# DiltheyLab/HLA-LA

Measured on AMD Instinct MI355X. Metric: paired reads/sec aligned to PRG graph, higher is better.
Workload: dtype int32

## Files before the change

hla-la_amd/__init__.py:

```python
from __future__ import annotations

import ctypes as C
import os

import numpy as np

_HERE = os.path.dirname(os.path.abspath(__file__))
LIB_PATH = os.environ.get("HLALA_LIB_PATH") or os.path.join(_HERE, "libhlala_gpu.so")

c_i32p = C.POINTER(C.c_int32)
c_i64p = C.POINTER(C.c_int64)
c_u8p = C.POINTER(C.c_uint8)
c_u32p = C.POINTER(C.c_uint32)
c_f64p = C.POINTER(C.c_double)

CHAIN_OK, CHAIN_SKIP_STRAND, CHAIN_SKIP_DUP = 0, 1, 2
CHAIN_ERR_COLUMNS, CHAIN_ERR_FRONTIER, CHAIN_ERR_INPUT = -1, -2, -3


class GraphDesc(C.Structure):
    _fields_ = [("n_levels", C.c_int32), ("n_nodes", C.c_int32), ("n_edges", C.c_int32),
                ("node_level", c_i32p), ("edge_from", c_i32p), ("edge_to", c_i32p), ("edge_label", c_u8p)]


# ... 163 lines not shown
    return _filter_call(lambda *a: fn(ctx.h, *a), "hlala_filter_positions_gpu", ctx.last_error, e, params, raw)


def filter_gpu_times(ctx, enable=True):
    ms = (C.c_double * 6)()
    ctx.lib.hlala_filter_gpu_times.argtypes = [C.c_void_p, C.c_int, C.POINTER(C.c_double)]
    if ctx.lib.hlala_filter_gpu_times(ctx.h, int(bool(enable)), ms) != 0:
        raise HlalaError("hlala_filter_gpu_times failed")
    return dict(zip(("mapq_keys", "sort_scan", "first20", "reads", "coverage", "use"), (float(x) for x in ms)))


def host_filter_model(e, params=None, tie_rule=0, raw=False):
    h = _host_lib()
    fn = h.hlala_host_filter_model
    fn.argtypes = [C.POINTER(ExonPositionsOut), C.POINTER(FilterParams), c_u8p, c_u8p, C.POINTER(FilterStats), C.POINTER(C.c_int64), C.c_int32]; fn.restype = C.c_int
    h.hlala_host_last_error.restype = C.c_char_p
    return _filter_call(lambda *a: fn(*a, int(tie_rule)), "hlala_host_filter_model", lambda: h.hlala_host_last_error().decode(errors="replace"), e, params, raw)


CALL_ORDER_MAX_HEAP = 4096
CALL_ORDER_TILE = 1024
CALL_ORDER_COUNTS = ("path", "levels", "tile_ranges", "largest_tile", "heap_sorts", "largest_heap", "bytes_up", "bytes_down")
CALL_ORDER_HOST, CALL_ORDER_DEVICE, CALL_ORDER_REFUSED_NAN, CALL_ORDER_REFUSED_HEAP, CALL_ORDER_REFUSED_ALLOC = range(5)


def call_order_params():
    v = [C.c_int32() for _ in range(4)]
    h = _host_lib(); h.hlala_host_pair_order_params.restype = None
    h.hlala_host_pair_order_params(*[C.byref(x) for x in v])
    return dict(zip(("tile", "max_heap", "block", "chunk"), (x.value for x in v)))


def _pair_order_call(call, what, last_error, ll, ma, raw):
    a = [np.ascontiguousarray(x, np.float64) for x in (ll, ma)]
    n = len(a[0]); assert len(a[1]) == n
    order = np.full(max(1, n), -7, np.int32); cn = (C.c_int64 * 8)()
    rc = call(n, a[0].ctypes.data_as(c_f64p), a[1].ctypes.data_as(c_f64p), order.ctypes.data_as(c_i32p), cn)
    out = (order[:n], dict(zip(CALL_ORDER_COUNTS, (int(x) for x in cn))))
    if raw:
        return (int(rc), last_error() if rc != 0 else "") + out
    if rc != 0:
        err = HlalaError(f"{what} failed ({rc}): {last_error()}"); err.code = int(rc)
        raise err
    return out


# ... 1362 lines not shown
```

hla-la_amd/csrc/batch.h:

```cpp
#pragma once
#include "device_common.h"

namespace hlala {

template <template <class> class Ptr> struct DevBatchT {
    int n_pairs, n_reads, n_chains, stride;
    int from_seeds;
    int unpaired;
    Ptr<const int> read_off;
    Ptr<const uint8_t> read_bases;
    Ptr<const uint8_t> read_quals;
    Ptr<const int> chain_off;
    Ptr<const int> read_primary;
    Ptr<const int> chain_read;
    Ptr<const int> chain_contig;
    Ptr<const int> chain_pos;
    Ptr<const int> chain_offset;
    Ptr<const int> chain_as;
    Ptr<const uint8_t> chain_reverse;
    Ptr<const int> cigar_off;
    Ptr<const u32> cigar;
    Ptr<int> seed_status;
    Ptr<int> seed_ncols;
    Ptr<int> seed_begin;
// ... 31 lines not shown
    Ptr<uint8_t> strands_valid;
    Ptr<uint8_t> sel_mapq;
    Ptr<u64> counters;
    Ptr<int> work_counter;
    Ptr<int> retry_list;
    Ptr<int> pair_multi;
    Ptr<uint8_t> pair_deferred;
    Ptr<int> chain_order;
    Ptr<int> chain_bucket;
    Ptr<int> order_hist;
    int order_shift, order_nb;
    int long_chunk_nodes, long_max_segs;
    int order_cost;
    Ptr<int> chain_row;
    int n_rows;
    Ptr<int> dp_blk;
    Ptr<int> dp_list;
    int dp_nblk;
    int dp_band;
    int dp_band_risky;
    int dp_band_nodes;
    int dp_jf;
    int dp_long;
    Ptr<void> dp_items;
    Ptr<int> dbg;
};
typedef DevBatchT<HostP> DevBatch;
typedef DevBatchT<GlobP> DevBatchG;
static_assert(sizeof(DevBatch) == sizeof(DevBatchG), "one layout");
__device__ __forceinline__ const DevBatchG& dev_view(const DevBatch* p) { return *(const DevBatchG*)p; }
enum { DESC_VALUE = 0, DESC_VIEW = 1, DESC_GENERIC = 2 };
template <int FORM, class D> __device__ __forceinline__ decltype(auto) desc_of(const D& byValue, const D* inMemory)
{
    if constexpr (FORM == DESC_VIEW) return dev_view(inMemory);
    else if constexpr (FORM == DESC_GENERIC) return (*inMemory);
    else return (byValue);
}

template <class BT> __device__ __forceinline__ int ordered_chains(const BT& B) { return B.chain_order ? __builtin_amdgcn_readfirstlane(B.order_hist[B.order_nb - 1]) : B.n_chains; }

template <class BT> __device__ __forceinline__ size_t row_base(const BT& B, int c) { return (size_t)(B.chain_row ? B.chain_row[c] : c) * (size_t)B.stride; }

enum { DPL_BAND16 = 0, DPL_BAND32 = 2, DPL_BAND64 = 4, DPL_JF = 6, DPL_GEN = 10, DPL_N = 14 };
__host__ __device__ inline int dpl_list(int cls, int dir, bool isLong)
{
    if(cls >= 2) return (cls == 2 ? DPL_BAND16 : (cls == 3 ? DPL_BAND32 : DPL_BAND64)) + dir;
// ... 18 lines not shown
```

hla-la_amd/csrc/hlala_api.hip:

```cpp
#include <cmath>
#include <cstdio>
#include <cstring>
#include <cstdlib>
#include <algorithm>
#include <atomic>
#include <map>
#include <mutex>
#include <chrono>
#include <thread>
#include <set>
#include <string>
#include <unordered_map>
#include <vector>

#include "../../include/hlala_gpu.h"
#include "batch.h"
#include "flat_graph.hpp"
#include "host_internal.h"

#include "kernel_dp.hip"
#include "kernel_project.hip"
#include "kernel_order.hip"
#include "kernel_pair.hip"
#include "kernel_pair_overflow.hip"
// ... 42 lines not shown
    hlala_params params{};
    FlatGraph F;
    DevGraph G{};
    DevGraph* dG = nullptr;
    DevTables* dT = nullptr;
    double* d_islog = nullptr;
    long long* d_contig_off = nullptr; uint8_t* d_contig_seq = nullptr; int* d_contig_level = nullptr;
    int n_contigs = 0; std::vector<long long> contig_off;
    std::vector<void*> allocs;
    std::unordered_map<void*, size_t> block_bytes;
    std::multimap<size_t, void*> pool;
    size_t pool_bytes = 0;
    size_t pool_cap = (size_t)176 << 30;
    std::mutex pool_mu;
    std::set<struct hlala_batch*> batches;
    int dp_long_bases = 48;
    int jf_margin = 16;
    int stitch_by_row = 1;
    int stitch_draw = 12;
    bool side_after_pair = false;
    bool rows_all = false;
    bool band_risky = false;
    bool band_nodes = true;
    int band_grid = 0, band_margin = 8;
    DpClass dp[DP_LAST_TIER + 1]; DpClass dp_jf;
    int stitch_grid = 0;
    char* proj_slabs = nullptr; size_t proj_slab_bytes = 0; int proj_grid = 0, pair_grid = 0, pair_lean_grid = 0;
    char* rethread_slabs = nullptr; size_t rethread_slab_bytes = 0; int rethread_grid = 0;
    double* pair_scratch = nullptr;
    char* pair_over_slabs = nullptr; long long pair_over_scratch = 0, pair_over_slab_bytes = 0;
    char* proj_long_slabs = nullptr; size_t proj_long_slab_bytes = 0;
    void* create_scratch = nullptr; size_t create_scratch_bytes = 0; bool create_scratch_pinned = false;
    int long_chunk_nodes = 1 << 20, long_max_segs = 1 << 20;
    int order_cost = 0;
    int order_shift = 8, order_nb = 0;
    int* dbg_host = nullptr;
    int* d_cov = nullptr; int n_cov = 0; int* d_gene_first = nullptr; int* d_gene_last = nullptr; int n_genes = 0;
    struct KeptReads { uint8_t* store = nullptr; long long* start = nullptr; int* length = nullptr; int n = 0; };
    std::vector<KeptReads> kept;
    bool flt_timed = false; double flt_ms[6] = {0, 0, 0, 0, 0, 0};
    bool ord_gpu = false, ord_timed = false; int64_t ord_counts[HLALA_CALL_ORDER_COUNTS] = {0, 0, 0, 0, 0, 0, 0, 0}; double ord_ms[4] = {0, 0, 0, 0};
    std::string err;
};

enum BatchEvent {
    EV_PROJECT_BEGIN, EV_PROJECT_END, EV_EXTEND_BEGIN, EV_EXTEND_END, EV_PAIR_BEGIN, EV_PAIR_END,
// ... 24 lines not shown
    uint32_t first_chain = 0;
    float ms[3] = {0, 0, 0};
};

struct DevGuard {
    int prev = -1, want = -1;
    explicit DevGuard(int device) : want(device) { if(device >= 0 && hipGetDevice(&prev) == hipSuccess && prev != device) (void)hipSetDevice(device); else prev = -1; }
    ~DevGuard() { if(prev >= 0 && prev != want) (void)hipSetDevice(prev); }
    DevGuard(const DevGuard&) = delete; DevGuard& operator=(const DevGuard&) = delete;
};
#define DEV_GUARD(c) DevGuard dev_guard_((c) ? (c)->device : -1)

#define HIP_TRY(ctx, call) do { hipError_t e_ = (call); if(e_ != hipSuccess) { (ctx)->err = std::string(#call) + ": " + hipGetErrorString(e_); return HLALA_E_DEVICE; } } while(0)
#define HIP_TRY_F(ctx, call, cleanup) do { hipError_t e_ = (call); if(e_ != hipSuccess) { (ctx)->err = std::string(#call) + ": " + hipGetErrorString(e_); return cleanup(HLALA_E_DEVICE); } } while(0)

template<class C, int TIER> static void launch_dp(hlala_ctx* c, const DpClass& k, hipStream_t ws, hlala_batch* b, const DpPoolArgs& pool)
{
    hipLaunchKernelGGL((k_dp<C, TIER>), dim3(k.grid), dim3(k.block), 0, ws, c->dG, b->dB, (DpItem*)b->B.dp_items, k.slabs, k.slab_bytes, c->params.rng_seed + 2u * b->first_chain,
                       c->G.nrec_out, c->G.nrec_in, b->B.read_bases, pool);
}
template<class C, int TIER> static DpClass dp_class(int grid, size_t slab_bytes, const char* name) { return DpClass{grid, C::THREADS, nullptr, slab_bytes, name, launch_dp<C, TIER>}; }

static int flush_tail(hlala_ctx* c);
static int join_side(hlala_ctx* c, hlala_batch* b)
{
    if(b->tail_pooled) { int rf = flush_tail(c); if(rf) return rf; }
    if(b->side_inflight) {
        HIP_TRY(c, hipStreamWaitEvent(c->stream, b->ev[EV_DONE], 0));
        if(b->ev[EV_MAIN]) { HIP_TRY(c, hipEventRecord(b->ev[EV_MAIN], c->stream)); b->mainValid = true; b->side_inflight = false; }
    }
    return HLALA_OK;
}
static int batch_events(hlala_ctx* c, hlala_batch* b)
{
    if(b->eventsMade) return HLALA_OK;
    for(int i = 0; i < EV_N; i++) HIP_TRY(c, hipEventCreateWithFlags(&b->ev[i], i < EV_TIMED_N ? hipEventDefault : hipEventDisableTiming));
    b->eventsMade = true;
    return HLALA_OK;
}
static int mark_main(hlala_ctx* c, hlala_batch* b) { HIP_TRY(c, hipEventRecord(b->ev[EV_MAIN], c->stream)); b->mainValid = true; return HLALA_OK; }
struct ReaderScope {
    hlala_ctx* c; int rc = HLALA_OK;
    ReaderScope(hlala_ctx* c_, hlala_batch* b) : c(c_)
    {
        if(!c) return;
        if(b && b->tail_pooled) { rc = flush_tail(c); if(rc) return; }
// ... 258 lines not shown
        rc = dev_upload(c, c->allocs, contigs->contig_seq, total, &c->d_contig_seq); if(rc) return fail(rc);
        rc = dev_upload(c, c->allocs, contigs->contig_level, total, &c->d_contig_level); if(rc) return fail(rc);
    }
    rc = build_tables(c); if(rc) return fail(rc);
    rc = dev_upload(c, c->allocs, &c->G, 1, &c->dG); if(rc) return fail(rc);
    hipDeviceProp_t prop;
    if(hipGetDeviceProperties(&prop, device) != hipSuccess) { c->err = "hipGetDeviceProperties failed"; return fail(HLALA_E_DEVICE); }
    int cus = prop.multiProcessorCount > 0 ? prop.multiProcessorCount : 256;
    auto slab_pool = [&](char** out, size_t bytes, const char* what) -> int {
        if(device_malloc_retry(c->device, nullptr, (void**)out, bytes) != hipSuccess) { c->err = std::string("hipMalloc(") + what + ") failed"; return HLALA_E_DEVICE; }
        c->allocs.push_back(*out);
        if(hipMemsetAsync(*out, 0, bytes, c->active) != hipSuccess) { c->err = std::string("hipMemset(") + what + ") failed"; return HLALA_E_DEVICE; }
        return 0;
    };
    c->band_grid = cus * 20;
    if(const char* e = getenv("HLALA_DP_BAND")) { if(atoi(e) == 0) c->band_grid = 0; }
    if(const char* e = getenv("HLALA_DP_BAND_RISKY")) c->band_risky = atoi(e) != 0;
    if(const char* e = getenv("HLALA_DP_BAND_NODES")) c->band_nodes = atoi(e) != 0;
    if(const char* e = getenv("HLALA_ROWS_ALL")) c->rows_all = atoi(e) != 0;
    if(const char* e = getenv("HLALA_SIDE_AFTER_PAIR")) c->side_after_pair = atoi(e) != 0;
    if(const char* e = getenv("HLALA_POOL_CAP_GB")) { const long g = atol(e); if(g >= 0 && g <= 1024) c->pool_cap = (size_t)g << 30; }
    if(const char* e = getenv("HLALA_DP_BAND_MARGIN")) { const int m = atoi(e); if(m >= 0 && m <= 24) c->band_margin = m; }
    if(const char* e = getenv("HLALA_DP_JF_MARGIN")) { const int m = atoi(e); if(m >= 0 && m <= 200) c->jf_margin = m; }
    if(const char* e = getenv("HLALA_DP_LONG_BASES")) { const int m = atoi(e); if(m >= 0 && m <= 4096) c->dp_long_bases = m; }
    c->stitch_grid = cus * 20;
    if(const char* e = getenv("HLALA_STITCH_BY_ROW")) c->stitch_by_row = atoi(e) != 0;
    const size_t extBytes = std::max(dp_slab_bytes<DpSmall>(), dp_slab_bytes<DpWide>()), largeBytes = std::max(dp_slab_bytes<DpLarge>(), dp_slab_bytes<DpBroad>());
    DpClass* const dp = c->dp;
    c->dp_jf = dp_class<DpTinyJF, 0>(cus * 4 * DpTinyJF::WAVES, dp_slab_bytes<DpTiny>(), "k_dp<DpTinyJF>");
    dp[0] = dp_class<DpTiny, 0>(cus * 4 * DpTiny::WAVES, dp_slab_bytes<DpTiny>(), "k_dp<DpTiny>");
    dp[1] = dp_class<DpMid, 1>(cus * 16, dp_slab_bytes<DpMid>(), "k_dp<DpMid>");
    dp[2] = dp_class<DpSmall, 2>(cus * 20, extBytes, "k_dp<DpSmall>");
    dp[3] = dp_class<DpWide, 3>(cus * 7, extBytes, "k_dp<DpWide>");
    dp[4] = dp_class<DpBroad, 4>(cus * 3, largeBytes, "k_dp<DpBroad>");
    dp[5] = dp_class<DpLarge, 5>(cus, largeBytes, "k_dp<DpLarge>");
    dp[6] = dp_class<DpHuge, 6>(cus / 4 > 0 ? cus / 4 : 1, dp_inmemory_bytes<DpHuge>(), "k_dp<DpHuge>");
    if((rc = slab_pool(&dp[0].slabs, dp[0].slab_bytes * (size_t)(64 / DpTiny::GW) * (size_t)std::max(dp[0].grid, c->dp_jf.grid), "16-lane DP slabs"))) return fail(rc);
    c->dp_jf.slabs = dp[0].slabs;
    if((rc = slab_pool(&dp[1].slabs, dp[1].slab_bytes * (size_t)(64 / DpMid::GW) * (size_t)dp[1].grid, "32-lane DP slabs"))) return fail(rc);
    if((rc = slab_pool(&dp[2].slabs, extBytes * (size_t)dp[2].grid, "64-lane DP slabs"))) return fail(rc);
    if((rc = slab_pool(&dp[3].slabs, extBytes * (size_t)dp[3].grid, "wide-class DP slabs"))) return fail(rc);
    if((rc = slab_pool(&dp[4].slabs, largeBytes * (size_t)(dp[4].grid + dp[5].grid), "large-class DP slabs"))) return fail(rc);
    dp[5].slabs = dp[4].slabs + largeBytes * (size_t)dp[4].grid;
    if((rc = slab_pool(&dp[6].slabs, dp[6].slab_bytes * (size_t)dp[6].grid, "in-memory DP class"))) return fail(rc);
    c->proj_grid = cus * (c->params.max_columns <= PROJ_CAP_SHORT ? 12 : 8); c->pair_grid = cus * 16; c->pair_lean_grid = cus * 24;
    { int rcp = dev_alloc(c, c->allocs, (size_t)2 * c->pair_grid * PAIR_COMB, &c->pair_scratch, false); if(rcp) return fail(rcp); }
// ... 94 lines not shown
static int batch_alloc_outputs(hlala_ctx* c, hlala_batch* b)
{
    DevBatch& B = b->B;
    size_t nc = (size_t)B.n_chains, nr = (size_t)B.n_reads, np = (size_t)B.n_pairs;
    if(!b->prepared) { B.n_rows = B.n_chains; B.chain_row = nullptr; }
    size_t rowsAlloc = (size_t)(B.n_rows > 0 ? B.n_rows : 1);
    if(b->prepared && nc >= 4096) { const size_t gran = nc / 64; rowsAlloc = (rowsAlloc + gran - 1) / gran * gran; if(rowsAlloc > nc) rowsAlloc = nc; }
    const size_t cs = rowsAlloc * (size_t)B.stride;
    int rc = 0;
#define AL(field, n, zero) do { rc = dev_alloc(c, b->allocs, (n), &B.field, zero); if(rc) return rc; } while(0)
    if(!b->prepared) { AL(seed_status, nc, true); AL(seed_ncols, nc, true); }
    AL(seed_begin, nc, true); AL(seed_end, nc, true); AL(seed_removed, nc, true);
    AL(seed_level, cs, false); AL(seed_edge, cs, false); AL(seed_g, cs, false); AL(seed_s, cs, false);
    AL(ext_status, nc, true); AL(ext_ncols, nc, true); AL(ext_begin, nc, true); AL(ext_end, nc, true); AL(ext_ll, nc, true);
    AL(dp_iters, 2 * nc, true); AL(dp_score, 2 * nc, true); AL(dp_ncols, 2 * nc, true); AL(dp_sb, 2 * nc, true); AL(dp_se, 2 * nc, true); AL(dp_err, 2 * nc, true);
    AL(dp_alias_head, 2 * nc, false); AL(dp_alias_next, 2 * nc, false);
    AL(ext_level, cs, false); AL(ext_edge, cs, false); AL(ext_g, cs, false); AL(ext_s, cs, false); AL(ext_fromseed, cs, false);
    AL(ext_firstlast, 4 * nc, true);
    AL(pair_status, np, true); AL(best_chain, nr, true); AL(n_comb, np, true); AL(pair_ll, np, true); AL(pair_mapq, np, true);
    AL(mate_mapq, nr, true); AL(strands_valid, np, true); AL(sel_mapq, nr * (size_t)B.stride, true);
    AL(pair_deferred, np, true); AL(pair_multi, 7 * np, false); AL(counters, 32, true); AL(work_counter, WC_N, true); AL(retry_list, 16 * nc, false);
    { DpItem* it = nullptr; rc = dev_alloc(c, b->allocs, 2 * nc, &it, false); if(rc) return rc; B.dp_items = it; }
    B.dp_nblk = (int)((nc + 255) / 256); if(B.dp_nblk < 1) B.dp_nblk = 1;
    B.dp_jf = c->jf_margin + 1; B.dp_long = c->dp_long_bases;
    B.dp_band = c->band_grid > 0 ? c->band_margin + 1 : 0;
    B.dp_band_risky = c->band_risky ? 1 : 0;
    B.dp_band_nodes = c->band_nodes ? 1 : 0;
    AL(dp_blk, (size_t)DPL_N * B.dp_nblk + 1, false); AL(dp_list, 2 * nc, false);
    if(!b->prepared) {
        B.chain_order = nullptr; B.chain_bucket = nullptr; B.order_hist = nullptr; B.order_shift = c->order_shift; B.order_nb = c->order_nb; B.order_cost = c->order_cost; B.long_chunk_nodes = c->long_chunk_nodes; B.long_max_segs = c->long_max_segs;
        if(c->order_nb > 0 && !B.from_seeds && nc > 0) { AL(chain_order, nc, false); AL(chain_bucket, nc, false); AL(order_hist, (size_t)c->order_nb + 1, false); }
    }
    B.dbg = c->dbg_host;
#undef AL
    return 0;
}

static int ctx_scratch(hlala_ctx* c, size_t need)
{
    if(need <= c->create_scratch_bytes) return HLALA_OK;
    if(c->create_scratch) { if(c->create_scratch_pinned) (void)hipHostFree(c->create_scratch); else free(c->create_scratch); c->create_scratch = nullptr; c->create_scratch_bytes = 0; }
    const size_t want = need + need / 8;
    void* p = nullptr;
    if(hipHostMalloc(&p, want, hipHostMallocDefault) == hipSuccess) c->create_scratch_pinned = true;
    else { (void)hipGetLastError(); p = malloc(want); c->create_scratch_pinned = false; }
    if(!p) { c->err = "out of host memory (batch scratch)"; return HLALA_E_ARG; }
    c->create_scratch = p; c->create_scratch_bytes = want;
    return HLALA_OK;
}

static int batch_create_tail(hlala_ctx* c, hlala_batch* b, std::chrono::steady_clock::time_point* queued)
// ... 259 lines not shown
        if(c->proj_long_slabs)
            hipLaunchKernelGGL((k_project_chains<ProjLdsLong>), dim3(grid), dim3(64), 0, c->active, c->G, b->B, c->dG, b->dB, c->d_contig_off, c->d_contig_seq, c->d_contig_level,
                               c->proj_slabs, c->proj_slab_bytes, c->proj_long_slabs, c->proj_long_slab_bytes, 0);
        else
            if(c->params.max_columns <= PROJ_CAP_SHORT)
                hipLaunchKernelGGL((k_project_chains<ProjLdsShort>), dim3(grid), dim3(64), 0, c->active, c->G, b->B, c->dG, b->dB, c->d_contig_off, c->d_contig_seq, c->d_contig_level,
                                   c->proj_slabs, c->proj_slab_bytes, (char*)nullptr, (size_t)0, c->rethread_slabs ? 1 : 0);
            else
                hipLaunchKernelGGL((k_project_chains<ProjLds>), dim3(grid), dim3(64), 0, c->active, c->G, b->B, c->dG, b->dB, c->d_contig_off, c->d_contig_seq, c->d_contig_level,
                               c->proj_slabs, c->proj_slab_bytes, (char*)nullptr, (size_t)0, c->rethread_slabs ? 1 : 0);
        int rc = check_launch(c, "k_project_chains"); if(rc) return rc;
        if(c->rethread_slabs) {
            hipLaunchKernelGGL(k_rethread_chains, dim3(c->rethread_grid), dim3(64), 0, c->active, c->dG, b->dB, c->rethread_slabs, c->rethread_slab_bytes);
            rc = check_launch(c, "k_rethread_chains"); if(rc) return rc;
        }
    }
    HIP_TRY(c, hipEventRecord(b->ev[EV_PROJECT_END], c->active));
    b->staged |= 1;
    return mark_main(c, b);
}

#define STEP(call) do { int rc_ = (call); if(rc_) return rc_; } while(0)
static bool fusable(const hlala_batch* b) { const DevBatch& B = b->B; return !(B.unpaired || B.from_seeds || B.n_pairs <= 0 || B.n_chains <= 0); }
static int dp_prepare(hlala_ctx* c, hlala_batch* b)
{
    DevBatch& B = b->B;
    b->side_used = false; b->side_pending = false;
    if(B.n_pairs > 0) HIP_TRY(c, hipMemsetAsync(B.pair_deferred, 0, (size_t)B.n_pairs, c->active));
    HIP_TRY(c, hipMemsetAsync(B.work_counter + 1, 0, sizeof(int), c->active));
    HIP_TRY(c, hipMemsetAsync(B.work_counter + 4, 0, (WC_N - 4) * sizeof(int), c->active));
    if(B.from_seeds) HIP_TRY(c, hipMemsetAsync(B.counters, 0, 32 * sizeof(u64), c->active));
    HIP_TRY(c, hipEventRecord(b->ev[EV_EXTEND_BEGIN], c->active));
    if(B.n_chains <= 0) return HLALA_OK;
    DpItem* items = (DpItem*)B.dp_items;
    HIP_TRY(c, hipMemsetAsync(B.dp_alias_head, 0xFF, (size_t)2 * B.n_chains * sizeof(int), c->active));
    HIP_TRY(c, hipMemsetAsync(B.dp_alias_next, 0xFF, (size_t)2 * B.n_chains * sizeof(int), c->active));
    HIP_TRY(c, hipMemsetAsync(B.dp_blk, 0, ((size_t)DPL_N * B.dp_nblk + 1) * sizeof(int), c->active));
    hipLaunchKernelGGL(k_dp_items, dim3(B.dp_nblk), dim3(256), 0, c->active, c->G, b->B, items);
    STEP(check_launch(c, "k_dp_items"));
    hipLaunchKernelGGL(k_order_scan, dim3(1), dim3(ORDER_SCAN_THREADS), 0, c->active, B.dp_blk, DPL_N * B.dp_nblk + 1);
    hipLaunchKernelGGL(k_dp_lists, dim3(B.dp_nblk), dim3(256), 0, c->active, b->B, (const DpItem*)items);
    return check_launch(c, "k_dp_lists");
}
static int dp_band(hlala_ctx* c, hlala_batch* b)
{
    DevBatch& B = b->B;
    b->band_used = c->band_grid > 0;
    if(!b->band_used) return HLALA_OK;
    const DpItem* items = (const DpItem*)B.dp_items; const u32 seed = c->params.rng_seed + 2u * b->first_chain;
    HIP_TRY(c, hipEventRecord(b->ev[EV_DP_BAND_BEGIN], c->active));
    hipLaunchKernelGGL((k_dp_band<16>), dim3(c->band_grid), dim3(64), 0, c->active, c->G, b->B, items, seed, (const uint8_t*)B.read_bases);
    hipLaunchKernelGGL((k_dp_band<32>), dim3(c->band_grid), dim3(64), 0, c->active, c->G, b->B, items, seed, (const uint8_t*)B.read_bases);
    hipLaunchKernelGGL((k_dp_band<64>), dim3(c->band_grid), dim3(64), 0, c->active, c->G, b->B, items, seed, (const uint8_t*)B.read_bases);
    STEP(check_launch(c, "k_dp_band"));
    HIP_TRY(c, hipEventRecord(b->ev[EV_DP_BAND_END], c->active)); return HLALA_OK;
}
static int dp_classes(hlala_ctx* c, hlala_batch* const* bs, int n, int first, int last, hipStream_t ws)
{
    const DpPoolArgs noPool{};
    DpPoolArgs pool{}; pool.n = n; hlala_batch* b0 = bs[0];
    for(int i = 0; i < n; i++) { const hlala_batch* b = bs[i]; pool.seed[i] = c->params.rng_seed + 2u * b->first_chain; pool.B[i] = b->dB; pool.items[i] = (const DpItem*)b->B.dp_items; pool.bases[i] = (const uint8_t*)b->B.read_bases; }
    for(int tier = first; tier <= last; tier++) {
        const DpClass& k = c->dp[tier];
        if(tier == 0) HIP_TRY(c, hipEventRecord(b0->ev[EV_DP_BEGIN], c->active));
        for(int i = 0; i < n; i++) HIP_TRY(c, hipEventRecord(bs[i]->ev[EV_DP_CLASS_BEGIN + tier], ws));
        if(tier == 0) {
            c->dp_jf.launch(c, c->dp_jf, ws, b0, noPool);
            STEP(check_launch(c, c->dp_jf.name));
            HIP_TRY(c, hipEventRecord(b0->ev[EV_DP_JUMP_FREE_END], ws));
        }
        k.launch(c, k, ws, b0, tier < DP_POOL_TIER ? noPool : pool);
        STEP(check_launch(c, k.name));
        for(int i = 0; i < n; i++) HIP_TRY(c, hipEventRecord(bs[i]->ev[EV_DP_CLASS_END + tier], ws));
        if(tier == 0 || tier == 2) HIP_TRY(c, hipEventRecord(b0->ev[tier == 0 ? EV_DP_CLASS0_END : EV_DP_CLASS2_END], c->active));
    }
    return HLALA_OK;
// ... 2873 lines not shown
```

hla-la_amd/csrc/host_check.cpp:

```cpp
#include <cstring>
#include <string>

#include "flat_graph.hpp"
#include "inflate_core.h"
#include "inflate_lds_model.h"
#include "crc32_core.h"
#include "bam_scan_model.h"
#include "bam_group_model.h"
#include "bam_nameorder_model.h"
#include "bam_fill_model.h"
#include "bam_resident_model.h"
#include "filter_gpu_model.h"
#include "call_order_model.h"

static thread_local std::string g_err;

extern "C" {
const char* hlala_host_last_error() { return g_err.c_str(); }

hlala::FlatGraph* hlala_host_flatten(const hlala_graph_desc* g, const hlala_contigs_desc* c)
{
    hlala::FlatGraph* F = new hlala::FlatGraph();
    g_err = hlala::flatten_graph(g, c, *F);
    if(!g_err.empty()) { delete F; return nullptr; }
    return F;
}
void hlala_host_free(hlala::FlatGraph* F) { delete F; }

int hlala_host_info(const hlala::FlatGraph* F, hlala_graph_info* info)
{
    memset(info, 0, sizeof(*info));
    info->n_levels = F->L; info->n_nodes = F->N; info->n_edges = F->E; info->n_paths = (int)F->path_len.size();
    info->n_jump_entries = (int64_t)F->jf_node.size(); info->n_path_edges = (int64_t)F->path_edges.size();
    info->n_levelpos_entries = (int64_t)F->lp_seqid.size();
    info->max_nodes_per_level = F->max_nodes_per_level; info->max_out_degree = F->max_out_degree; info->max_in_degree = F->max_in_degree; info->max_jumps = F->max_jumps; info->max_parallel = F->max_parallel;
    for(uint8_t b : F->gap_stretch) info->n_gap_stretch_levels += b;
// ... 148 lines not shown
    try { rc = hlala_order::pair_order_model(n, ll, ma, order, counts, &why); }
    catch(const std::exception&) { why = "out of memory"; rc = HLALA_E_ARG; }
    g_err = why.empty() ? std::string() : (why.rfind("not available:", 0) == 0 ? why : "hlala_host_pair_order_model: " + why);
    return rc;
}
int hlala_host_pair_order_reference(int64_t n, const double* ll, const double* ma, int32_t* order)
{
    if(const char* bad = hlala_order::ord_check_args(n, ll, ma, order)) { g_err = std::string("hlala_host_pair_order_reference: ") + bad; return HLALA_E_ARG; }
    try { hlala_order::pair_order_reference(n, ll, ma, order); }
    catch(const std::exception&) { g_err = "hlala_host_pair_order_reference: out of memory"; return HLALA_E_ARG; }
    g_err.clear();
    return HLALA_OK;
}
void hlala_host_pair_order_params(int32_t* tile, int32_t* max_heap, int32_t* block, int32_t* chunk)
{
    *tile = (int32_t)hlala_order::ORD_TILE; *max_heap = (int32_t)hlala_order::ORD_MAX_HEAP; *block = (int32_t)hlala_order::ORD_BLOCK; *chunk = (int32_t)hlala_order::ORD_CHUNK;
}
int hlala_host_batch_resident_model(const hlala_batch_in* in, int32_t n_contigs, int32_t unpaired, int32_t* read_off32, int32_t* chain_off32, int32_t* primary32, int32_t* chain_read,
                                    int32_t* cigar_off32, int64_t first[5])
{
    int64_t spare[hlala_bamres::RES_CLASSES];
    return hlala_bamres::resident_model(in, n_contigs, unpaired != 0, read_off32, chain_off32, primary32, chain_read, cigar_off32, first ? first : spare, &g_err);
}
}
```

hla-la_amd/csrc/kernel_dp.hip:

```cpp
#include "batch.h"
#include "../../include/hlala_gpu.h"

namespace hlala {

enum { K_DIAG = 0, K_GGAP = 1, K_SGAP = 2, K_HOP = 3, K_JUMP = 4 };
enum { M_D = 0, M_GG = 1, M_SG = 2 };
enum { PH_IDLE = 0, PH_RUN, PH_SELECT, PH_BT, PH_EXPAND, PH_DONE };

constexpr u64 HKEY_EMPTY = ~0ull;
#ifndef HLALA_DP_PROFILE_LOG2
#define HLALA_DP_PROFILE_LOG2 18
#endif
#ifndef HLALA_EARLY_GEN_MAX
#define HLALA_EARLY_GEN_MAX 0xFFFFFE
#endif
constexpr int DP_EARLY_GEN_MAX = HLALA_EARLY_GEN_MAX;
constexpr int EXT_PENDING = 0x7FFFFFFF;
constexpr int DP_BT_STEPS_PER_TRIP = 32;

#ifndef HLALA_DP_TAIL_THREADS
#define HLALA_DP_TAIL_THREADS 128
#endif
constexpr int DP_TAIL_THREADS = HLALA_DP_TAIL_THREADS;
#ifndef HLALA_DP_TINY_WAVES
// ... 1456 lines not shown
#define DP_T(i) do { } while(0)
#endif

    constexpr int NPASS = (TIER == 0 && !C::JF) ? 4 : 2;
    for(int pass = 0; pass < NPASS; pass++) {
        const int dirPass = pass & 1;
        const bool foPass = pass >= 2;
        constexpr int RT = TIER > 0 ? TIER : 1;
        int* fetchCounter = foPass ? &B.work_counter[WC_FO_FETCH + dirPass]
                          : &B.work_counter[TIER == 0 ? (C::JF ? 4 + dirPass : (dirPass ? 10 : 1)) : wc_retry_fetch(RT, dirPass)];
        const int seg = (C::JF ? DPL_JF : DPL_GEN) + 2 * dirPass;
        const bool dense = TIER == 0 && !foPass;
        const bool twoEnded = TIER > 0;
        const int segStart = dense ? uni(B.dp_blk[(size_t)seg * B.dp_nblk]) : 0;
        const int nLong = twoEnded ? uni(B.work_counter[wc_retry_long(RT, dirPass)]) : 0;
        const int nItems = dense ? uni(B.dp_blk[(size_t)(seg + 2) * B.dp_nblk]) - segStart
                         : (foPass ? uni(B.work_counter[WC_FO_COUNT + dirPass]) : nLong + uni(B.work_counter[wc_retry_short(RT, dirPass)]));
        const int nChains = B.n_chains;
        const int* srcList = dense ? B.dp_list + segStart
                           : (foPass ? B.retry_list + (size_t)(14 + dirPass) * (size_t)B.n_chains
                           : B.retry_list + (size_t)(2 * (RT - 1) + dirPass) * (size_t)B.n_chains);
        const bool fwd = dirPass != 0;
        if constexpr (DRAW > 1) { if(gl == 0) { S.chunkNext = 0; S.chunkEnd = 0; } DSYNC(); }
        int phase = PH_IDLE;
        bool more = true;
        int edgesAcc = 0;

        for(;;) {
            if(phase == PH_RUN) phase = dp_iterate<C>(S, sl, G, fwd ? nrecOut : nrecIn, readBases, fwd, edgesAcc, sortScratch);
            DP_T(5);
            if(phase == PH_SELECT) phase = dp_select<C>(S, sl, G, rng_seed, fwd);
            DP_T(4);
            if(phase == PH_BT) phase = dp_backtrace<C>(S, sl, DP_BT_STEPS_PER_TRIP, fwd);
            DP_T(3);
            if(phase == PH_EXPAND) phase = dp_expand<C>(S, sl, G, B, fwd ? nrecOut : nrecIn, fwd);
            DP_T(2);
            if(phase == PH_DONE) {
                const int edges = grp_sum_i32<GW>(edgesAcc);
                if(gl == 0) {
                    DpState& st = S.st;
                    S.nextPhase = PH_IDLE;
#ifdef HLALA_DP_PROFILE
                    if(B.dbg && TIER == HLALA_DP_PROFILE && !C::JF) {
                        const long long cyc = clock64() - S.pfStart;
                        if(cyc > (1ll << HLALA_DP_PROFILE_LOG2) && (HLALA_DP_PROFILE_LOG2 >= 12 || (((u32)st.item * 2654435761u) >> 24) == 0)) { int q = atomicAdd(&B.dbg[0], 1); if(q < 500) { int* r = B.dbg + 16 + 16 * q; r[0] = st.item; r[1] = st.itersRun; r[2] = (int)st.cellsEvaluated; r[3] = st.nCells;
                            r[4] = S.pfSlow; r[5] = S.pfImp; r[6] = S.pfPre; r[7] = (int)(cyc >> 10); r[8] = S.pfMaxNT;
// ... 24 lines not shown
                        int nx = B.dp_alias_head[item]; if(nx < 0) nx = B.dp_alias_next[item];
                        const bool failed = st.err != 0 && st.err > -1000000;
                        while(nx >= 0 && failed) {
                            B.dp_iters[nx] = st.itersRun; B.dp_score[nx] = INT32_MIN; B.dp_ncols[nx] = -1; B.dp_sb[nx] = st.sb; B.dp_se[nx] = st.se; B.dp_err[nx] = st.err;
                            S.accCalls++; S.accIters += (u64)st.itersRun; S.accCells += (u64)st.cellsEvaluated; S.accEdges += (u64)edges;
                            nx = B.dp_alias_next[nx];
                        }
                        if(nx >= 0) {
                            st.item = nx; st.isAlias = 1;
                            st.endSlot = -1; st.endScore = 0; st.nSteps = 0; st.nCols = 0; st.have = 0; st.sb = 0; st.se = -1; st.err = 0;
                            S.nextPhase = PH_SELECT;
                        }
                    }
                }
                DSYNC();
                phase = guni<GW>(S.nextPhase);
            }
            DP_T(1);
            if(phase == PH_IDLE && more) {
                int w = 0;
                if(gl == 0) {
                    if constexpr (DRAW > 1) {
                        int nx = S.chunkNext;
                        if(nx >= S.chunkEnd) { nx = atomicAdd(fetchCounter, DRAW); S.chunkEnd = nx + DRAW; }
                        S.chunkNext = nx + 1; w = nx;
                    } else w = atomicAdd(fetchCounter, 1);
                }
                w = grp_bcast0<GW>(w);
                if(w >= nItems) more = false;
                else {
                    const int idx = guni<GW>(srcList[twoEnded ? retry_entry(w, nLong, nChains) : w]);
                    const int4* ip = (const int4*)(items + idx);
                    int4 a = ip[0], b = ip[1];
                    DpItem it; it.item = a.x; it.rOff = a.y; it.seqLen = a.z; it.start_seq = a.w; it.startLevel = b.x; it.startNode = b.y; it.pad0 = 0; it.pad1 = 0;
                    phase = dp_begin<C>(S, sl, G, it, idx);
                    edgesAcc = 0;
                }
            }
            DP_T(0);
            if(!__ballot(phase != PH_IDLE)) break;
#ifdef HLALA_DP_TIMING
            trips++; runGroups += __popcll(__ballot(phase == PH_RUN)) / GW;
#endif
            DP_T(5);
        }
    }
    if(gl == 0 && S.accCalls) {
// ... 199 lines not shown
```

hla-la_amd/csrc/kernel_dp_band.hip:

```cpp
#include "batch.h"

namespace hlala {

constexpr int BAND_ABSENT = -20000;
constexpr int BAND_DRAW = 16;
constexpr int BAND_TIES = 16;

template <int GW_> struct BandCfg;
template <> struct BandCfg<16> { static constexpr int GW = 16, MAXJ = BAND_MAXJ16, REACH = 64, MAXD = 96, WAVES = 5; };
template <> struct BandCfg<32> { static constexpr int GW = 32, MAXJ = BAND_MAXJ32, REACH = 96, MAXD = 128, WAVES = 5; };
template <> struct BandCfg<64> { static constexpr int GW = 64, MAXJ = BAND_MAXJ64, REACH = 112, MAXD = 160, WAVES = 5; };

template <class C>
struct __align__(16) BandLds {
    u32 bt[C::MAXD / 8][C::GW];
    unsigned short steps[C::MAXD];
    unsigned short tieD[BAND_TIES];
    u32 ls[C::REACH];
};

template <int GW> __device__ __forceinline__ int band_prev(int v, int gl)
{
    if(GW == 16) return dpp_mov<0x111>(DP_NEG, v);
    int r = __builtin_amdgcn_update_dpp(DP_NEG, v, 0x138, 0xF, 0xF, false);
// ... 4 lines not shown
#ifdef HLALA_BAND_TIMING
#define BAND_T(i) do { __builtin_amdgcn_s_waitcnt(0); const long long t_ = clock64(); tAcc[i] += t_ - tMark; tMark = t_; } while(0)
#else
#define BAND_T(i) do { } while(0)
#endif

template <class C, bool FWD, class DG, class DB>
__device__ __forceinline__ void band_pass(const DG& G, const DB& B, const DpItem* __restrict__ items, const u32 rng_seed, const uint8_t* __restrict__ readBases,
                                          BandLds<C>& S, u64& accCalls, u64& accIters, u64& accCells, u64& accEdges)
{
    constexpr int GW = C::GW, NG = 64 / GW;
    const int lane = lane_id(), g = lane / GW, gl = lane & (GW - 1), rowBase = lane & ~(GW - 1);
    constexpr int dirPass = FWD ? 1 : 0;
    constexpr int listK = (GW == 16 ? DPL_BAND16 : (GW == 32 ? DPL_BAND32 : DPL_BAND64)) + dirPass;
    const int segStart = uni(B.dp_blk[(size_t)listK * B.dp_nblk]);
    const int nItems = uni(B.dp_blk[(size_t)(listK + 1) * B.dp_nblk]) - segStart;
    const int* srcList = B.dp_list + segStart;
    int* fetchCounter = &B.work_counter[WC_BAND_FETCH + (GW == 16 ? 0 : (GW == 32 ? 2 : 4)) + dirPass];
    const int stride = B.stride;
    const int levelsL = G.L;
#ifdef HLALA_BAND_TIMING
    long long tAcc[6] = {0, 0, 0, 0, 0, 0}; long long tMark = clock64();
#endif
    int chunkNext = 0, chunkEnd = 0;
    for(;;) {
        BAND_T(4);
        if(chunkNext >= chunkEnd) {
            int w0 = 0;
            if(lane == 0) w0 = atomicAdd(fetchCounter, NG * BAND_DRAW);
            chunkNext = __builtin_amdgcn_readfirstlane(w0); chunkEnd = chunkNext + NG * BAND_DRAW;
        }
        if(chunkNext >= nItems) break;
        const int w = chunkNext + g;
        chunkNext += NG;
        const bool has = w < nItems;
        int idx = 0; int4 a = make_int4(-1, 0, 0, 0), b4 = make_int4(0, 0, 0, 0);
        if(has) { idx = srcList[w]; const int4* ip = (const int4*)(items + idx); a = ip[0]; b4 = ip[1]; }
        const int item0 = a.x, rOff = a.y, seqLen = a.z, y0 = a.w, x0 = b4.x;
        const int linRun = (b4.z >> 8) & 255, pos0 = b4.w;
        const int jmax = has ? (FWD ? seqLen - y0 : y0) : 0;
        const int reach = min(linRun, C::REACH);
        int myRc = 0;
        if(has) {
            for(int t = gl; t < reach; t += GW) S.ls[t] = (FWD ? G.npf_label : G.npb_label)[pos0 + t];
            if(gl >= 1 && gl <= jmax) myRc = readBases[rOff + (FWD ? y0 + gl - 1 : y0 - gl)];
        }
        const u32 rcRep = (u32)myRc * 0x01010101u;
        WSYNC();
        BAND_T(0);

        int D1 = (has && gl == 0) ? 0 : DP_NEG, G1 = DP_NEG, S1 = DP_NEG, D2 = DP_NEG;
        int curMax = 0, lastInc = 0, firstPos = 0;
        int cBest = DP_NEG, cCount = 0, cFirstD = 0;
        u32 btAcc = 0;
        int cellsAcc = 0, edgesAcc = 0, itersRun = 0;
// ... 151 lines not shown
                nx = B.dp_alias_head[item]; if(nx < 0) nx = B.dp_alias_next[item];
#endif
            }
            nx = __shfl(nx, rowBase);
            if(nx < 0) live = false; else item = nx;
            first = false;
            BAND_T(3);
        }
        if(has && fail && gl == 0) {
            const int q = atomicAdd(&B.work_counter[WC_FO_COUNT + dirPass], 1);
            B.retry_list[(size_t)(14 + dirPass) * (size_t)B.n_chains + q] = idx;
            atomicAdd(&B.work_counter[WC_BAND_FAILED], 1); atomicAdd(&B.work_counter[WC_BAND_WHY + fail], 1);
        }
        WSYNC();
#ifdef HLALA_BAND_TIMING
        tAcc[4] += 0; if(lane == 0) atomicAdd(&B.counters[22], 1ull);
#endif
    }
#ifdef HLALA_BAND_TIMING
    if(lane == 0 && GW == 16) { for(int i = 0; i < 5; i++) atomicAdd(&B.counters[16 + i], (u64)tAcc[i]); atomicAdd(&B.counters[21], (u64)tAcc[5]); }
#endif
}

template <int GW>
__global__ __launch_bounds__(64, BandCfg<GW>::WAVES) void k_dp_band(const DevGraph G, const DevBatch B, const DpItem* __restrict__ items, const u32 rng_seed,
                                                                    const uint8_t* __restrict__ readBases)
{
    typedef BandCfg<GW> C;
    __shared__ BandLds<C> SS[64 / GW];
    BandLds<C>& S = SS[lane_id() / GW];
    u64 accCalls = 0, accIters = 0, accCells = 0, accEdges = 0;
    band_pass<C, false>(G, B, items, rng_seed, readBases, S, accCalls, accIters, accCells, accEdges);
    band_pass<C, true>(G, B, items, rng_seed, readBases, S, accCalls, accIters, accCells, accEdges);
    if((lane_id() & (GW - 1)) == 0 && accCalls) {
        atomicAdd(&B.counters[CNT_DP_CALLS], accCalls); atomicAdd(&B.counters[CNT_DP_ITERS], accIters);
        atomicAdd(&B.counters[CNT_DP_CELLS], accCells); atomicAdd(&B.counters[CNT_EDGES], accEdges);
    }
}

}
```

hla-la_amd/csrc/kernel_order.hip:

```cpp
#include "batch.h"

namespace hlala {

constexpr int ORDER_SCAN_THREADS = 1024;

__global__ __launch_bounds__(ORDER_SCAN_THREADS) void k_order_scan(int* hist, int nb)
{
    __shared__ int part[ORDER_SCAN_THREADS];
    const int t = threadIdx.x;
    const int per = (nb + ORDER_SCAN_THREADS - 1) / ORDER_SCAN_THREADS;
    const int a = t * per, z = min(nb, a + per);
    int s = 0;
    for(int i = a; i < z; i++) s += hist[i];
    part[t] = s;
    __syncthreads();
    for(int o = 1; o < ORDER_SCAN_THREADS; o <<= 1) {
        const int v = t >= o ? part[t - o] : 0;
        __syncthreads();
        part[t] += v;
        __syncthreads();
    }
    int run = part[t] - s;
    for(int i = a; i < z; i++) { const int h = hist[i]; hist[i] = run; run += h; }
}

__global__ void k_order_scatter(const DevBatch* __restrict__ Bp)
{
    const DevBatch& B = *Bp;
    const int c = blockIdx.x * blockDim.x + threadIdx.x;
    if(c >= B.n_chains) return;
    const int bk = B.chain_bucket[c];
    if(bk < 0) { if(B.chain_row) B.chain_row[c] = -1; return; }
    const int pos = atomicAdd(&B.order_hist[bk], 1);
    B.chain_order[pos] = c;
    if(B.chain_row) B.chain_row[c] = pos;
}

__global__ void k_unpack_bases(const uint8_t* __restrict__ packed, const int* __restrict__ read_off, const int n_reads, const long long rb0, const long long firstRead,
                               const long long p0, uint8_t* __restrict__ out)
{
    const int r = blockIdx.x;
    if(r >= n_reads) return;
    const int o0 = read_off[r], len = read_off[r + 1] - o0;
    const long long at = ((rb0 + (long long)o0 + firstRead + (long long)r + 1) >> 1) - p0;
    auto dec = [](unsigned c) -> uint8_t {
        const u32 w = c < 4 ? 0x4D43413Du : (c < 8 ? 0x56535247u : (c < 12 ? 0x48595754u : 0x4E42444Bu));
// ... 11 lines not shown
```

Before: 5.829 million.

## Taper DP work draws, fuse band kernels, and tile the DP list scan

Work fetching in the DP and band kernels now draws chunked units for the body of the item list and single items for a tail window, so load balances better at the end of the pass. The three band kernels (widths 16/32/64) are fused into one launch that shares LDS through a union and runs all passes in sequence. The single-block prefix scan over the DP list histogram is replaced by a three-kernel multi-block tiled scan. These aim to cut tail idle time, launch gaps and a serial scan, but the fused band kernel runs the classes in a fixed order inside each block, which may reduce overlap between them.

```diff
diff --git a/hla-la_amd/__init__.py b/hla-la_amd/__init__.py
--- a/hla-la_amd/__init__.py
+++ b/hla-la_amd/__init__.py
@@ -209,6 +209,22 @@
 CALL_ORDER_TILE = 1024
 CALL_ORDER_COUNTS = ("path", "levels", "tile_ranges", "largest_tile", "heap_sorts", "largest_heap", "bytes_up", "bytes_down")
 CALL_ORDER_HOST, CALL_ORDER_DEVICE, CALL_ORDER_REFUSED_NAN, CALL_ORDER_REFUSED_HEAP, CALL_ORDER_REFUSED_ALLOC = range(5)
+
+
+def dp_draw_units(n, window, draw, cap):
+    h = _host_lib()
+    first = np.zeros(cap, np.int32); count = np.zeros(cap, np.int32)
+    h.hlala_host_dp_draw_units.restype = C.c_int
+    h.hlala_host_dp_draw_units.argtypes = [C.c_int32] * 4 + [C.c_void_p] * 2
+    u = h.hlala_host_dp_draw_units(int(n), int(window), int(draw), int(cap), first.ctypes.data, count.ctypes.data)
+    if u < 0:
+        raise ValueError("dp_draw_units(%d, %d, %d, %d): bad arguments" % (n, window, draw, cap))
+    return u, first, count
+
+
+def dp_draw_window(n, per_drawer, drawers, items=-1):
+    h = _host_lib(); h.hlala_host_dp_draw_window.restype = C.c_int; h.hlala_host_dp_draw_window.argtypes = [C.c_int32] * 4
+    return h.hlala_host_dp_draw_window(int(n), int(per_drawer), int(drawers), int(items))
 
 
 def call_order_params():
diff --git a/hla-la_amd/csrc/batch.h b/hla-la_amd/csrc/batch.h
--- a/hla-la_amd/csrc/batch.h
+++ b/hla-la_amd/csrc/batch.h
@@ -1,5 +1,6 @@
 #pragma once
 #include "device_common.h"
+#include "dp_draw_core.h"
 
 namespace hlala {
 
@@ -77,6 +78,8 @@
     int dp_band_nodes;
     int dp_jf;
     int dp_long;
+    int dp_taper;
+    int dp_taper_items;
     Ptr<void> dp_items;
     Ptr<int> dbg;
 };
diff --git a/hla-la_amd/csrc/dp_draw_core.h b/hla-la_amd/csrc/dp_draw_core.h
--- /dev/null
+++ b/hla-la_amd/csrc/dp_draw_core.h
@@ -0,0 +1,33 @@
+#ifndef HLALA_DP_DRAW_CORE_H_
+#define HLALA_DP_DRAW_CORE_H_
+
+#ifndef HLALA_HD
+#ifdef __HIPCC__
+#define HLALA_HD __host__ __device__ inline
+#else
+#define HLALA_HD inline
+#endif
+#endif
+
+namespace hlala_draw {
+
+HLALA_HD int draw_window(int n, int perDrawer, int drawers, int items)
+{
+    long long t = items >= 0 ? (long long)items : (long long)perDrawer * (long long)drawers;
+    if(t < 0) t = 0;
+    return t > (long long)n ? (n > 0 ? n : 0) : (int)t;
+}
+
+HLALA_HD int draw_body_units(int n, int T, int D) { return (int)(((long long)(n - T) + D - 1) / D); }
+
+HLALA_HD bool draw_unit(int w, int n, int T, int D, int* first, int* count)
+{
+    const int body = n - T, U1 = draw_body_units(n, T, D);
+    if(w >= 0 && w < U1) { const long long a = (long long)w * D; *first = (int)a; *count = (int)((a + D < (long long)body ? a + D : (long long)body) - a); return true; }
+    if(w >= U1 && (long long)w - U1 < (long long)T) { *first = body + (w - U1); *count = 1; return true; }
+    *first = n > 0 ? n : 0; *count = 0;
+    return false;
+}
+
+}
+#endif
diff --git a/hla-la_amd/csrc/hlala_api.hip b/hla-la_amd/csrc/hlala_api.hip
--- a/hla-la_amd/csrc/hlala_api.hip
+++ b/hla-la_amd/csrc/hlala_api.hip
@@ -88,6 +88,9 @@
     bool rows_all = false;
     bool band_risky = false;
     bool band_nodes = true;
+    int dp_taper = 4, dp_taper_items = -1;
+    bool band_fused = true;
+    int dp_scan_tile = 1024;
     int band_grid = 0, band_margin = 8;
     DpClass dp[DP_LAST_TIER + 1]; DpClass dp_jf;
     int stitch_grid = 0;
@@ -158,6 +161,7 @@
 template<class C, int TIER> static DpClass dp_class(int grid, size_t slab_bytes, const char* name) { return DpClass{grid, C::THREADS, nullptr, slab_bytes, name, launch_dp<C, TIER>}; }
 
 static int flush_tail(hlala_ctx* c);
+static int dp_scan_tiles(const hlala_ctx* c, int nb);
 static int join_side(hlala_ctx* c, hlala_batch* b)
 {
     if(b->tail_pooled) { int rf = flush_tail(c); if(rf) return rf; }
@@ -462,6 +466,10 @@
     if(const char* e = getenv("HLALA_POOL_CAP_GB")) { const long g = atol(e); if(g >= 0 && g <= 1024) c->pool_cap = (size_t)g << 30; }
     if(const char* e = getenv("HLALA_DP_BAND_MARGIN")) { const int m = atoi(e); if(m >= 0 && m <= 24) c->band_margin = m; }
     if(const char* e = getenv("HLALA_DP_JF_MARGIN")) { const int m = atoi(e); if(m >= 0 && m <= 200) c->jf_margin = m; }
+    if(const char* e = getenv("HLALA_DP_BAND_FUSED")) c->band_fused = atoi(e) != 0;
+    if(const char* e = getenv("HLALA_DP_TAPER")) { const int m = atoi(e); if(m >= 0 && m <= 4096) c->dp_taper = m; }
+    if(const char* e = getenv("HLALA_DP_TAPER_ITEMS")) { const int m = atoi(e); if(m >= 0) c->dp_taper_items = m; }
+    if(const char* e = getenv("HLALA_DP_SCAN_TILE")) { const int m = atoi(e); if(m == 0 || (m >= 16 && m <= 65536)) c->dp_scan_tile = m; }
     if(const char* e = getenv("HLALA_DP_LONG_BASES")) { const int m = atoi(e); if(m >= 0 && m <= 4096) c->dp_long_bases = m; }
     c->stitch_grid = cus * 20;
     if(const char* e = getenv("HLALA_STITCH_BY_ROW")) c->stitch_by_row = atoi(e) != 0;
@@ -602,11 +610,11 @@
     AL(pair_deferred, np, true); AL(pair_multi, 7 * np, false); AL(counters, 32, true); AL(work_counter, WC_N, true); AL(retry_list, 16 * nc, false);
     { DpItem* it = nullptr; rc = dev_alloc(c, b->allocs, 2 * nc, &it, false); if(rc) return rc; B.dp_items = it; }
     B.dp_nblk = (int)((nc + 255) / 256); if(B.dp_nblk < 1) B.dp_nblk = 1;
-    B.dp_jf = c->jf_margin + 1; B.dp_long = c->dp_long_bases;
+    B.dp_jf = c->jf_margin + 1; B.dp_long = c->dp_long_bases; B.dp_taper = c->dp_taper; B.dp_taper_items = c->dp_taper_items;
     B.dp_band = c->band_grid > 0 ? c->band_margin + 1 : 0;
     B.dp_band_risky = c->band_risky ? 1 : 0;
     B.dp_band_nodes = c->band_nodes ? 1 : 0;
-    AL(dp_blk, (size_t)DPL_N * B.dp_nblk + 1, false); AL(dp_list, 2 * nc, false);
+    AL(dp_blk, (size_t)DPL_N * B.dp_nblk + 1 + dp_scan_tiles(c, DPL_N * B.dp_nblk + 1), false); AL(dp_list, 2 * nc, false);
     if(!b->prepared) {
         B.chain_order = nullptr; B.chain_bucket = nullptr; B.order_hist = nullptr; B.order_shift = c->order_shift; B.order_nb = c->order_nb; B.order_cost = c->order_cost; B.long_chunk_nodes = c->long_chunk_nodes; B.long_max_segs = c->long_max_segs;
         if(c->order_nb > 0 && !B.from_seeds && nc > 0) { AL(chain_order, nc, false); AL(chain_bucket, nc, false); AL(order_hist, (size_t)c->order_nb + 1, false); }
@@ -912,6 +920,7 @@
 
 #define STEP(call) do { int rc_ = (call); if(rc_) return rc_; } while(0)
 static bool fusable(const hlala_batch* b) { const DevBatch& B = b->B; return !(B.unpaired || B.from_seeds || B.n_pairs <= 0 || B.n_chains <= 0); }
+static int dp_scan_tiles(const hlala_ctx* c, int nb) { return c->dp_scan_tile > 0 ? (nb + c->dp_scan_tile - 1) / c->dp_scan_tile : 0; }
 static int dp_prepare(hlala_ctx* c, hlala_batch* b)
 {
     DevBatch& B = b->B;
@@ -928,7 +937,17 @@
     HIP_TRY(c, hipMemsetAsync(B.dp_blk, 0, ((size_t)DPL_N * B.dp_nblk + 1) * sizeof(int), c->active));
     hipLaunchKernelGGL(k_dp_items, dim3(B.dp_nblk), dim3(256), 0, c->active, c->G, b->B, items);
     STEP(check_launch(c, "k_dp_items"));
-    hipLaunchKernelGGL(k_order_scan, dim3(1), dim3(ORDER_SCAN_THREADS), 0, c->active, B.dp_blk, DPL_N * B.dp_nblk + 1);
+    {
+        const int nb = DPL_N * B.dp_nblk + 1, nTiles = dp_scan_tiles(c, nb);
+        int* sums = B.dp_blk + nb;
+        if(nTiles == 0) hipLaunchKernelGGL(k_order_scan, dim3(1), dim3(ORDER_SCAN_THREADS), 0, c->active, B.dp_blk, nb);
+        else {
+            hipLaunchKernelGGL(k_scan_tile_sums, dim3(nTiles), dim3(SCAN_TILE_THREADS), 0, c->active, (const int*)B.dp_blk, nb, c->dp_scan_tile, sums);
+            hipLaunchKernelGGL(k_scan_tile_offsets, dim3(1), dim3(SCAN_TILE_THREADS), 0, c->active, sums, nTiles);
+            hipLaunchKernelGGL(k_scan_tiles, dim3(nTiles), dim3(SCAN_TILE_THREADS), 0, c->active, B.dp_blk, nb, c->dp_scan_tile, (const int*)sums);
+        }
+        STEP(check_launch(c, "dp_prepare: scan"));
+    }
     hipLaunchKernelGGL(k_dp_lists, dim3(B.dp_nblk), dim3(256), 0, c->active, b->B, (const DpItem*)items);
     return check_launch(c, "k_dp_lists");
 }
@@ -939,9 +958,12 @@
     if(!b->band_used) return HLALA_OK;
     const DpItem* items = (const DpItem*)B.dp_items; const u32 seed = c->params.rng_seed + 2u * b->first_chain;
     HIP_TRY(c, hipEventRecord(b->ev[EV_DP_BAND_BEGIN], c->active));
+    if(c->band_fused) hipLaunchKernelGGL(k_dp_band_all, dim3(c->band_grid), dim3(64), 0, c->active, c->G, b->B, items, seed, (const uint8_t*)B.read_bases);
+    else {
     hipLaunchKernelGGL((k_dp_band<16>), dim3(c->band_grid), dim3(64), 0, c->active, c->G, b->B, items, seed, (const uint8_t*)B.read_bases);
     hipLaunchKernelGGL((k_dp_band<32>), dim3(c->band_grid), dim3(64), 0, c->active, c->G, b->B, items, seed, (const uint8_t*)B.read_bases);
     hipLaunchKernelGGL((k_dp_band<64>), dim3(c->band_grid), dim3(64), 0, c->active, c->G, b->B, items, seed, (const uint8_t*)B.read_bases);
+    }
     STEP(check_launch(c, "k_dp_band"));
     HIP_TRY(c, hipEventRecord(b->ev[EV_DP_BAND_END], c->active)); return HLALA_OK;
 }
diff --git a/hla-la_amd/csrc/host_check.cpp b/hla-la_amd/csrc/host_check.cpp
--- a/hla-la_amd/csrc/host_check.cpp
+++ b/hla-la_amd/csrc/host_check.cpp
@@ -12,6 +12,7 @@
 #include "bam_resident_model.h"
 #include "filter_gpu_model.h"
 #include "call_order_model.h"
+#include "dp_draw_core.h"
 
 static thread_local std::string g_err;
 
@@ -206,4 +207,11 @@
     int64_t spare[hlala_bamres::RES_CLASSES];
     return hlala_bamres::resident_model(in, n_contigs, unpaired != 0, read_off32, chain_off32, primary32, chain_read, cigar_off32, first ? first : spare, &g_err);
 }
-}
+int hlala_host_dp_draw_units(int32_t n, int32_t T, int32_t D, int32_t cap, int32_t* first, int32_t* count)
+{
+    if(n < 0 || T < 0 || T > n || D < 1 || cap < 0 || (cap && (!first || !count))) return -1;
+    for(int32_t w = 0; w < cap; w++) { int f = 0, k = 0; hlala_draw::draw_unit(w, n, T, D, &f, &k); first[w] = f; count[w] = k; }
+    return hlala_draw::draw_body_units(n, T, D) + T;
+}
+int hlala_host_dp_draw_window(int32_t n, int32_t perDrawer, int32_t drawers, int32_t items) { return hlala_draw::draw_window(n, perDrawer, drawers, items); }
+}
diff --git a/hla-la_amd/csrc/kernel_dp.hip b/hla-la_amd/csrc/kernel_dp.hip
--- a/hla-la_amd/csrc/kernel_dp.hip
+++ b/hla-la_amd/csrc/kernel_dp.hip
@@ -1502,6 +1502,7 @@
                            : B.retry_list + (size_t)(2 * (RT - 1) + dirPass) * (size_t)B.n_chains);
         const bool fwd = dirPass != 0;
         if constexpr (DRAW > 1) { if(gl == 0) { S.chunkNext = 0; S.chunkEnd = 0; } DSYNC(); }
+        const int window = DRAW > 1 ? hlala_draw::draw_window(nItems, B.dp_taper, (int)gridDim.x * NG, B.dp_taper_items) : 0;
         int phase = PH_IDLE;
         bool more = true;
         int edgesAcc = 0;
@@ -1572,7 +1573,11 @@
                 if(gl == 0) {
                     if constexpr (DRAW > 1) {
                         int nx = S.chunkNext;
-                        if(nx >= S.chunkEnd) { nx = atomicAdd(fetchCounter, DRAW); S.chunkEnd = nx + DRAW; }
+                        if(nx >= S.chunkEnd) {
+                            int uFirst = 0, uCount = 0;
+                            hlala_draw::draw_unit(atomicAdd(fetchCounter, 1), nItems, window, DRAW, &uFirst, &uCount);
+                            nx = uFirst; S.chunkEnd = uFirst + uCount;
+                        }
                         S.chunkNext = nx + 1; w = nx;
                     } else w = atomicAdd(fetchCounter, 1);
                 }
diff --git a/hla-la_amd/csrc/kernel_dp_band.hip b/hla-la_amd/csrc/kernel_dp_band.hip
--- a/hla-la_amd/csrc/kernel_dp_band.hip
+++ b/hla-la_amd/csrc/kernel_dp_band.hip
@@ -50,15 +50,17 @@
 #ifdef HLALA_BAND_TIMING
     long long tAcc[6] = {0, 0, 0, 0, 0, 0}; long long tMark = clock64();
 #endif
+    const int nTasks = (nItems + NG - 1) / NG;
+    const int window = hlala_draw::draw_window(nTasks, B.dp_taper, (int)gridDim.x, B.dp_taper_items);
     int chunkNext = 0, chunkEnd = 0;
     for(;;) {
         BAND_T(4);
         if(chunkNext >= chunkEnd) {
-            int w0 = 0;
-            if(lane == 0) w0 = atomicAdd(fetchCounter, NG * BAND_DRAW);
-            chunkNext = __builtin_amdgcn_readfirstlane(w0); chunkEnd = chunkNext + NG * BAND_DRAW;
-        }
-        if(chunkNext >= nItems) break;
+            int w0 = 0, uFirst = 0, uCount = 0;
+            if(lane == 0) w0 = atomicAdd(fetchCounter, 1);
+            if(!hlala_draw::draw_unit(__builtin_amdgcn_readfirstlane(w0), nTasks, window, BAND_DRAW, &uFirst, &uCount)) break;
+            chunkNext = uFirst * NG; chunkEnd = chunkNext + uCount * NG;
+        }
         const int w = chunkNext + g;
         chunkNext += NG;
         const bool has = w < nItems;
@@ -256,6 +258,16 @@
 #endif
 }
 
+__device__ __forceinline__ void band_tail_clock(const DevBatch& B, const int ki)
+{
+#if defined(HLALA_DP_TIMING) && HLALA_DP_TIMING + 0 == 2
+    if(lane_id() == 0) {
+        const u64 now = (u64)wall_clock64();
+        atomicMax((unsigned long long*)&B.counters[16 + 2 * ki], (unsigned long long)~now); atomicMax((unsigned long long*)&B.counters[17 + 2 * ki], (unsigned long long)now);
+    }
+#endif
+}
+
 template <int GW>
 __global__ __launch_bounds__(64, BandCfg<GW>::WAVES) void k_dp_band(const DevGraph G, const DevBatch B, const DpItem* __restrict__ items, const u32 rng_seed,
                                                                     const uint8_t* __restrict__ readBases)
@@ -270,6 +282,32 @@
         atomicAdd(&B.counters[CNT_DP_CALLS], accCalls); atomicAdd(&B.counters[CNT_DP_ITERS], accIters);
         atomicAdd(&B.counters[CNT_DP_CELLS], accCells); atomicAdd(&B.counters[CNT_EDGES], accEdges);
     }
-}
-
-}
+    band_tail_clock(B, GW == 16 ? 5 : (GW == 32 ? 6 : 7));
+}
+
+union BandLdsAll {
+    BandLds<BandCfg<64>> s64[1];
+    BandLds<BandCfg<32>> s32[2];
+    BandLds<BandCfg<16>> s16[4];
+};
+static_assert(BandCfg<16>::WAVES == 5 && BandCfg<32>::WAVES == 5 && BandCfg<64>::WAVES == 5, "k_dp_band_all: one launch bound");
+
+__global__ __launch_bounds__(64, 5) void k_dp_band_all(const DevGraph G, const DevBatch B, const DpItem* __restrict__ items, const u32 rng_seed, const uint8_t* __restrict__ readBases)
+{
+    __shared__ BandLdsAll SS;
+    const int lane = lane_id();
+    u64 accCalls = 0, accIters = 0, accCells = 0, accEdges = 0;
+    band_pass<BandCfg<64>, false>(G, B, items, rng_seed, readBases, SS.s64[0], accCalls, accIters, accCells, accEdges);
+    band_pass<BandCfg<64>, true>(G, B, items, rng_seed, readBases, SS.s64[0], accCalls, accIters, accCells, accEdges);
+    band_pass<BandCfg<32>, false>(G, B, items, rng_seed, readBases, SS.s32[lane / 32], accCalls, accIters, accCells, accEdges);
+    band_pass<BandCfg<32>, true>(G, B, items, rng_seed, readBases, SS.s32[lane / 32], accCalls, accIters, accCells, accEdges);
+    band_pass<BandCfg<16>, false>(G, B, items, rng_seed, readBases, SS.s16[lane / 16], accCalls, accIters, accCells, accEdges);
+    band_pass<BandCfg<16>, true>(G, B, items, rng_seed, readBases, SS.s16[lane / 16], accCalls, accIters, accCells, accEdges);
+    if((lane & 15) == 0 && accCalls) {
+        atomicAdd(&B.counters[CNT_DP_CALLS], accCalls); atomicAdd(&B.counters[CNT_DP_ITERS], accIters);
+        atomicAdd(&B.counters[CNT_DP_CELLS], accCells); atomicAdd(&B.counters[CNT_EDGES], accEdges);
+    }
+    band_tail_clock(B, 5);
+}
+
+}
diff --git a/hla-la_amd/csrc/kernel_order.hip b/hla-la_amd/csrc/kernel_order.hip
--- a/hla-la_amd/csrc/kernel_order.hip
+++ b/hla-la_amd/csrc/kernel_order.hip
@@ -22,6 +22,60 @@
     }
     int run = part[t] - s;
     for(int i = a; i < z; i++) { const int h = hist[i]; hist[i] = run; run += h; }
+}
+
+constexpr int SCAN_TILE_THREADS = 256;
+
+__device__ __forceinline__ int block_excl_scan(const int v, int* part, int& total)
+{
+    constexpr int NW = SCAN_TILE_THREADS / 64;
+    int wtot; const int x = wave_excl_scan(v, wtot);
+    const int wv = (int)threadIdx.x >> 6;
+    __syncthreads();
+    if(lane_id() == 0) part[wv] = wtot;
+    __syncthreads();
+    int before = 0, all = 0;
+#pragma unroll
+    for(int k = 0; k < NW; k++) { const int p = part[k]; if(k < wv) before += p; all += p; }
+    total = all;
+    return before + x;
+}
+
+__global__ __launch_bounds__(SCAN_TILE_THREADS) void k_scan_tile_sums(const int* __restrict__ hist, const int nb, const int tile, int* __restrict__ sums)
+{
+    __shared__ int part[SCAN_TILE_THREADS / 64];
+    const long long a = (long long)blockIdx.x * tile; const int z = (int)min((long long)nb, a + tile);
+    int s = 0;
+    for(int i = (int)a + (int)threadIdx.x; i < z; i += SCAN_TILE_THREADS) s += hist[i];
+    int total; (void)block_excl_scan(s, part, total);
+    if(threadIdx.x == 0) sums[blockIdx.x] = total;
+}
+
+__global__ __launch_bounds__(SCAN_TILE_THREADS) void k_scan_tile_offsets(int* sums, const int nTiles)
+{
+    __shared__ int part[SCAN_TILE_THREADS / 64];
+    int run = 0;
+    for(int i0 = 0; i0 < nTiles; i0 += SCAN_TILE_THREADS) {
+        const int i = i0 + (int)threadIdx.x;
+        const int v = i < nTiles ? sums[i] : 0;
+        int total; const int x = block_excl_scan(v, part, total);
+        if(i < nTiles) sums[i] = run + x;
+        run += total;
+    }
+}
+
+__global__ __launch_bounds__(SCAN_TILE_THREADS) void k_scan_tiles(int* hist, const int nb, const int tile, const int* __restrict__ sums)
+{
+    __shared__ int part[SCAN_TILE_THREADS / 64];
+    const long long a = (long long)blockIdx.x * tile; const int z = (int)min((long long)nb, a + tile);
+    int run = sums[blockIdx.x];
+    for(int i0 = (int)a; i0 < z; i0 += SCAN_TILE_THREADS) {
+        const int i = i0 + (int)threadIdx.x;
+        const int v = i < z ? hist[i] : 0;
+        int total; const int x = block_excl_scan(v, part, total);
+        if(i < z) hist[i] = run + x;
+        run += total;
+    }
 }
 
 __global__ void k_order_scatter(const DevBatch* __restrict__ Bp)
```

After: 5.856 million, median of 6. No clear change (+0.5%).
